# vovw/algonauts-2025

Hardware: AMD Instinct MI355X
Metric: TRs/sec trimodal encode to 1000 parcels (higher is better)
Workload: dtype bf16; 1 GPU; trimodal encode, precomputed bf16 feats, per GPU B=64 sequences (4 subjects x R=16) x T=1024, L*D=4096 per modality, hidden 3072, 8 layers, V=1000 parcels, n_output_timesteps=1024; forward only; global_batch=64, seq_len=1024, parallelism=dp1

## Files before the change

### algonauts-2025_amd/csrc/attention.hip

```cpp
#include "attn_common.h"
#include "attn_acc_regs.h"
#include "host_plan.h"

namespace {

template <int DH>
struct AttnCfg {
  static constexpr int NSUB = DH <= 64 ? 4 : (DH <= 128 ? 2 : 1);
  static constexpr int KS = DH / 32;
  static constexpr int DT = DH / 16;
  static constexpr int ROWB = DH * 2;
  static constexpr int KV = 32 * NSUB;
  static constexpr int TILE_BYTES = KV * ROWB;
  static constexpr int CHUNKS = DH / 8;
  static constexpr int WAVES = 8;
  static constexpr int PIECES = KV * CHUNKS / 64;
  static constexpr int PPW = (PIECES + WAVES - 1) / WAVES;
  static constexpr int SWZ_MASK = (CHUNKS % 16 == 0) ? 15 : 7;
  static constexpr int NBUF = DH >= 192 ? 3 : 2;
  static constexpr int SMEM = NBUF * 2 * TILE_BYTES;
  static_assert(DH % 64 == 0, "dim_head must be a multiple of 64");
};

template <int DH>
// ... 117 lines not shown
#pragma unroll
        for (int j = 0; j < 8; ++j) sv[u][j] = -INFINITY;
        continue;
      }
      f32x4_t s0 = {0.f, 0.f, 0.f, 0.f}, s1 = {0.f, 0.f, 0.f, 0.f};
#pragma unroll
      for (int ks = 0; ks < C::KS; ++ks) {
        const int off = k_rd[ks % KRD] + (ks / KRD) * SEG * 16 + u * 32 * C::ROWB;
        const bf16x8_t ka = *(const bf16x8_t*)(kt + off);
        const bf16x8_t kb2 = *(const bf16x8_t*)(kt + off + 16 * C::ROWB);
        s0 = __builtin_amdgcn_mfma_f32_16x16x32_bf16(ka, qf[ks], s0, 0, 0, 0);
        s1 = __builtin_amdgcn_mfma_f32_16x16x32_bf16(kb2, qf[ks], s1, 0, 0, 0);
      }
      const int key_base = sub_key0 + 4 * fq;
      if (RELKEY) {
        const float* qrow_e = a.qe + ((int64_t)b * T + qrow) * a.ld_qe + h * a.qe_stride_h + a.rel_left;
#pragma unroll
        for (int r = 0; r < 4; ++r) {
          int d0 = key_base + r - qrow, d1 = key_base + 16 + r - qrow;
          d0 = d0 < -a.rel_left ? -a.rel_left : (d0 > a.rel_right ? a.rel_right : d0);
          d1 = d1 < -a.rel_left ? -a.rel_left : (d1 > a.rel_right ? a.rel_right : d1);
          s0[r] += qrow_e[d0];
          s1[r] += qrow_e[d1];
        }
      }
      const bool edge = sub_key0 + 32 > T || (CAUSAL && sub_key0 + 31 > q0);
      if (edge) {
#pragma unroll
        for (int r = 0; r < 4; ++r) {
          sv[u][r] = (key_base + r < lim) ? s0[r] : -INFINITY;
          sv[u][4 + r] = (key_base + 16 + r < lim) ? s1[r] : -INFINITY;
        }
      } else {
#pragma unroll
        for (int r = 0; r < 4; ++r) { sv[u][r] = s0[r]; sv[u][4 + r] = s1[r]; }
      }
      pmax = fmaxf(pmax, fmaxf(sv[u][0], sv[u][4]));
#pragma unroll
      for (int r = 1; r < 4; ++r) pmax = max3f(pmax, sv[u][r], sv[u][4 + r]);
    }
    pmax = fmaxf(pmax, __shfl_xor(pmax, 16, 64));
    pmax = fmaxf(pmax, __shfl_xor(pmax, 32, 64));
    pmax *= scale_log2e;
    if (!__all(pmax - m_run <= 8.0f)) {
      const float m_new = fmaxf(m_run, pmax);
      const float alpha = __builtin_amdgcn_exp2f(m_run - m_new);
      m_run = m_new;
      l_run *= alpha;
      if (LSUM_MFMA) {
#pragma unroll
        for (int r = 0; r < 4; ++r) lacc[r] *= alpha;
      }
#pragma unroll
      for (int dt = 0; dt < C::DT; ++dt)
#pragma unroll
        for (int r = 0; r < 4; ++r) o[dt][r] *= alpha;
    }
    bf16x8_t pf[C::NSUB];
    float psum = 0.f;
#pragma unroll
    for (int u = 0; u < C::NSUB; ++u)
#pragma unroll
      for (int j = 0; j < 8; ++j) {
        const float p = __builtin_amdgcn_exp2f(fmaf(sv[u][j], scale_log2e, -m_run));
        if (!LSUM_MFMA) psum += p;
        pf[u][j] = (short)f32_to_bf16(p);
      }
    l_run += psum;

#pragma unroll
    for (int u = 0; u < C::NSUB; ++u) {
      const int sub_key0 = t * C::KV + u * 32;
      if (sub_key0 >= T || (CAUSAL && sub_key0 > q0 + 15)) continue;
      if (LSUM_MFMA) lacc = __builtin_amdgcn_mfma_f32_16x16x32_bf16(ones, pf[u], lacc, 0, 0, 0);
#pragma unroll
      for (int dt = 0; dt < C::DT; ++dt) {
        const int off = v_rd[dt % VRD] + (dt / VRD) * SEG * 16 + u * 32 * C::ROWB;
        const s16x4_t lo = __builtin_amdgcn_ds_read_tr16_b64_v4i16((__attribute__((address_space(3))) s16x4_t*)(vt + off));
        const s16x4_t hi =
            __builtin_amdgcn_ds_read_tr16_b64_v4i16((__attribute__((address_space(3))) s16x4_t*)(vt + off + 16 * C::ROWB));
        bf16x8_t vf;
#pragma unroll
        for (int e = 0; e < 4; ++e) { vf[e] = lo[e]; vf[4 + e] = hi[e]; }
        o[dt] = __builtin_amdgcn_mfma_f32_16x16x32_bf16(vf, pf[u], o[dt], 0, 0, 0);
      }
    }
    }
    if (C::NBUF == 3) {
      asm volatile("s_waitcnt lgkmcnt(0)" ::: "memory");
      if (t + 2 < ntiles) { stage((t + 2) % C::NBUF, (t + 2) * C::KV); wait_keep_one_tile(); }
      else { asm volatile("s_waitcnt vmcnt(0)" ::: "memory"); }
      __builtin_amdgcn_s_barrier();
    } else {
      asm volatile("s_waitcnt vmcnt(0)" ::: "memory");
      __syncthreads();
    }
  }

  float l_tot;
  if (LSUM_MFMA) {
    l_tot = lacc[0];
  } else {
    l_tot = l_run + __shfl_xor(l_run, 16, 64);
    l_tot += __shfl_xor(l_tot, 32, 64);
  }
  const float inv = 1.0f / l_tot;
  const int q = q0 + l15;
  if (q < T) {
    unsigned short* orow = a.out + ((int64_t)b * T + q) * a.ld_out + (int64_t)h * DH + 4 * fq;
#pragma unroll
    for (int dt = 0; dt < C::DT; ++dt) {
      u16x4_t pk;
#pragma unroll
      for (int e = 0; e < 4; ++e) pk[e] = f32_to_bf16(o[dt][e] * inv);
      *(u16x4_t*)(orow + 16 * dt) = pk;
    }
  }
}


struct WideCfg {
  static constexpr int DH = 384, KS = 24, DT = 12, ROWB = 768, KV = 32, CHUNKS = 48;
  static constexpr int TILE_BYTES = KV * ROWB;
  static constexpr int WAVES = 4, PPW = 6;
  static constexpr int K_SLOTS = 2, V_SLOTS = 4;
  static constexpr int V_BASE = K_SLOTS * TILE_BYTES;
  static constexpr int SMEM = (K_SLOTS + V_SLOTS) * TILE_BYTES;
  static constexpr int DEPTH = 6;
};

__device__ __forceinline__ int swz_wide(int chunk, int row) {
  return (chunk & ~15) | ((chunk ^ (((row & 3) << 2) | ((row >> 2) & 3))) & 15);
}


__device__ __forceinline__ void mfma_s_first(f32x16_t& acc, const bf16x8_t& a, const bf16x8_t& b) {
  asm volatile("v_mfma_f32_32x32x16_bf16 %0, %1, %2, 0" : "=&v"(acc) : "v"(a), "v"(b));
}
__device__ __forceinline__ void mfma_s(f32x16_t& acc, const bf16x8_t& a, const bf16x8_t& b) {
  asm volatile("v_mfma_f32_32x32x16_bf16 %0, %1, %2, %0" : "+v"(acc) : "v"(a), "v"(b));
}


__global__ __launch_bounds__(256, 1) void attn_fwd_wide384_kernel(const AttnArgs a) {
  using C = WideCfg;
  extern __shared__ __attribute__((aligned(16))) char smem[];
  const int tid = threadIdx.x, lane = tid & 63;
  const int wave = __builtin_amdgcn_readfirstlane(tid >> 6);
  const int r31 = lane & 31, h = lane >> 5;

  const int T = a.T;
  const float scale_log2e = a.scale_log2e;
  const int xcd = blockIdx.x & 7, slot = blockIdx.x >> 3;
  const int qb = slot % a.qblocks;
  const int pair = (slot / a.qblocks) * 8 + xcd;
  if (pair >= a.n_bh) return;
  const int hd = pair % a.heads_q;
  const int b = pair / a.heads_q;
  const int hk = hd / a.group;
  const int64_t ld = a.ld_kv;
  const unsigned short* qbase = a.q + (int64_t)b * T * a.ld_q + (int64_t)hd * C::DH;
  const unsigned short* kbase = a.k + (int64_t)b * T * ld + (int64_t)hk * C::DH;
  const unsigned short* vbase = a.v + (int64_t)b * T * ld + (int64_t)hk * C::DH;

  const int q0 = qb * 128 + wave * 32;
  const int qrow = (q0 + r31 < T) ? q0 + r31 : T - 1;
  bf16x8_t qf[C::KS];
#pragma unroll
  for (int ks = 0; ks < C::KS; ++ks) qf[ks] = *(const bf16x8_t*)(qbase + (int64_t)qrow * a.ld_q + ks * 16 + h * 8);
  if (a.q_cos) {
    const int half = a.q_rot_dim >> 1;
    const float* cr = a.q_cos + (int64_t)qrow * half;
    const float* sr = a.q_sin + (int64_t)qrow * half;
#pragma unroll
    for (int ks = 0; ks < C::KS; ++ks) {
      const int d0 = ks * 16 + h * 8;
      if (d0 < a.q_rot_dim) {
        const float4 c4 = *(const float4*)(cr + (d0 >> 1)), s4 = *(const float4*)(sr + (d0 >> 1));
        const float cs[4] = {c4.x, c4.y, c4.z, c4.w}, sn[4] = {s4.x, s4.y, s4.z, s4.w};
#pragma unroll
        for (int pp = 0; pp < 4; ++pp) {
          const float qa = bf16_to_f32((unsigned short)qf[ks][2 * pp]), qb = bf16_to_f32((unsigned short)qf[ks][2 * pp + 1]);
          qf[ks][2 * pp] = (short)f32_to_bf16(qa * cs[pp] - qb * sn[pp]);
          qf[ks][2 * pp + 1] = (short)f32_to_bf16(qb * cs[pp] + qa * sn[pp]);
        }
      }
    }
  }

  int st_row[C::PPW], st_src[C::PPW], st_off[C::PPW];
#pragma unroll
  for (int i = 0; i < C::PPW; ++i) {
    const int p = (wave + C::WAVES * i) * 64 + lane;
    st_row[i] = p / C::CHUNKS;
    st_src[i] = swz_wide(p % C::CHUNKS, st_row[i]) * 8;
    st_off[i] = st_row[i] * (int)ld + st_src[i];
  }
  const unsigned lds0_u = __builtin_amdgcn_readfirstlane(lds_addr(smem));
  auto stage_piece = [&](int which, int slot, int key0, int i) {
    const char* sbase = (const char*)((which ? vbase : kbase) + (int64_t)key0 * ld);
    const int piece = wave + C::WAVES * i;
    unsigned voff = (unsigned)st_off[i] * 2u;
    if (key0 + C::KV > T) {
      const int row = (key0 + st_row[i] < T) ? st_row[i] : T - 1 - key0;
      voff = (unsigned)(row * (int)ld + st_src[i]) * 2u;
    }
    const unsigned dst = lds0_u + (which ? C::V_BASE : 0) + slot * C::TILE_BYTES + piece * 1024;
    asm volatile("s_mov_b32 m0, %0\n\ts_nop 0\n\tglobal_load_lds_dwordx4 %1, %2" : : "s"(dst), "v"(voff), "s"(sbase) : "memory");
  };
  auto stage = [&](int which, int slot, int key0) {
#pragma unroll
    for (int i = 0; i < C::PPW; ++i) stage_piece(which, slot, key0, i);
  };

  int kb_off[8];
#pragma unroll
  for (int i = 0; i < 8; ++i) kb_off[i] = r31 * C::ROWB + swz_wide(2 * i + h, r31) * 16;
  const int tq = (lane & 15) >> 2, tp = lane & 3, g1 = (lane >> 4) & 1;
  int vb_off[4][2];
#pragma unroll
  for (int i = 0; i < 4; ++i)
#pragma unroll
    for (int lh = 0; lh < 2; ++lh) {
      const int row = 4 * h + tq + 8 * lh;
      vb_off[i][lh] = C::V_BASE + row * C::ROWB + swz_wide(4 * i + 2 * g1 + (tp >> 1), row) * 16 + (tp & 1) * 8;
    }
  auto ld_k = [&](const int (&ka)[8], int ks) -> bf16x8_t {
    return *(const bf16x8_t*)(smem + ka[ks & 7] + (ks >> 3) * 256);
  };
  auto ld_v = [&](const int (&va)[4][2], int i) -> bf16x8_t {
    const int s = i / C::DT, dt = i % C::DT;
    const int imm = (dt >> 2) * 256 + s * 16 * C::ROWB;
    const s16x4_t lo = __builtin_amdgcn_ds_read_tr16_b64_v4i16((__attribute__((address_space(3))) s16x4_t*)(smem + va[dt & 3][0] + imm));
    const s16x4_t hi = __builtin_amdgcn_ds_read_tr16_b64_v4i16((__attribute__((address_space(3))) s16x4_t*)(smem + va[dt & 3][1] + imm));
    bf16x8_t vf;
#pragma unroll
    for (int e = 0; e < 4; ++e) { vf[e] = lo[e]; vf[4 + e] = hi[e]; }
    return vf;
  };

  static_for<0, C::DT>([&](auto dt) { AccTile<decltype(dt)::value>::zero(); });
  float m_run = -INFINITY, l_run = 0.f;

  const int ntiles = (T + C::KV - 1) / C::KV;
  stage(0, 0, 0); stage(1, 0, 0);
  if (ntiles > 1) { stage(0, 1, C::KV); stage(1, 1, C::KV); asm volatile("s_waitcnt vmcnt(12)" ::: "memory"); }
  else { asm volatile("s_waitcnt vmcnt(0)" ::: "memory"); }
  __builtin_amdgcn_s_barrier();

  bf16x8_t kf[C::KS], vf[2 * C::DT];
  int ka[8], va[4][2];
#pragma unroll
  for (int i = 0; i < 8; ++i) ka[i] = kb_off[i];
#pragma unroll
  for (int i = 0; i < 4; ++i) { va[i][0] = vb_off[i][0]; va[i][1] = vb_off[i][1]; }
#pragma unroll
  for (int d = 0; d < C::DEPTH; ++d) kf[d] = ld_k(ka, d);

#ifdef TRIBE_ATTN_STAMPS
  unsigned long long ts0 = 0, ts1 = 0, ts2 = 0, ts3 = 0, ts4 = 0, ts5 = 0;
  unsigned long long stamp_acc[5] = {0, 0, 0, 0, 0};
#endif
  int vcur = 0;
  for (int t = 0; t < ntiles; ++t) {
    ATTN_STAMP(ts0);
    const bool more = t + 2 < ntiles;
    const int vnext2 = (vcur + 2) & 3;

    f32x16_t s;
#pragma unroll
    for (int ks = 0; ks < C::KS; ++ks) {
      if (ks + C::DEPTH < C::KS) kf[ks + C::DEPTH] = ld_k(ka, ks + C::DEPTH);
      else vf[ks + C::DEPTH - C::KS] = ld_v(va, ks + C::DEPTH - C::KS);
      if (ks % 4 == 1) { if (more) stage_piece(1, vnext2, (t + 2) * C::KV, ks / 4); }
      __builtin_amdgcn_sched_barrier(0);
      if (ks == 0) mfma_s_first(s, kf[ks], qf[ks]);
      else mfma_s(s, kf[ks], qf[ks]);
      __builtin_amdgcn_sched_barrier(0);
    }
    asm volatile("s_nop 11" : "+v"(s));
    ATTN_STAMP(ts1);

    if ((t + 1) * C::KV > T) {
#pragma unroll
      for (int r = 0; r < 16; ++r)
        if (t * C::KV + (r & 3) + 8 * (r >> 2) + 4 * h >= T) s[r] = -INFINITY;
    }
    float pmax = max3f(s[0], s[1], s[2]);
#pragma unroll
    for (int r = 3; r < 15; r += 2) pmax = max3f(pmax, s[r], s[r + 1]);
    pmax = fmaxf(pmax, s[15]);
    pmax = pair_max(pmax) * scale_log2e;
    if (!__all(pmax - m_run <= 8.0f)) {
      const float m_new = fmaxf(m_run, pmax);
      const float alpha = __builtin_amdgcn_exp2f(m_run - m_new);
      m_run = m_new;
      l_run *= alpha;
      if (t > 0) {
        asm volatile("s_nop 15\n\ts_nop 7" ::: "memory");
        static_for<0, C::DT>([&](auto dt) { AccTile<decltype(dt)::value>::scale(alpha); });
        asm volatile("s_nop 7" ::: "memory");
      }
    }
    bf16x8_t pf[2];
    float psum = 0.f;
#pragma unroll
    for (int r = 0; r < 16; ++r) {
      const float p = __builtin_amdgcn_exp2f(fmaf(s[r], scale_log2e, -m_run));
      psum += p;
      pf[r >> 3][r & 7] = (short)f32_to_bf16(p);
    }
    l_run += psum;

    ATTN_STAMP(ts2);
    if (more) asm volatile("s_waitcnt vmcnt(6)" ::: "memory");
    else asm volatile("s_waitcnt vmcnt(0)" ::: "memory");
    ATTN_STAMP(ts3);
    __builtin_amdgcn_s_barrier();
    ATTN_STAMP(ts4);
    const int kslot = t & 1;
    const int kstep = kslot ? -C::TILE_BYTES : C::TILE_BYTES;
#pragma unroll
    for (int i = 0; i < 8; ++i) asm volatile("v_add_u32 %0, %1, %0" : "+v"(ka[i]) : "s"(kstep));
    asm volatile("s_nop 1" : "+v"(pf[0]), "+v"(pf[1]));

    static_for<0, 2 * C::DT>([&](auto ic) {
      constexpr int i = decltype(ic)::value;
      if constexpr (i + C::DEPTH < 2 * C::DT) vf[i + C::DEPTH] = ld_v(va, i + C::DEPTH);
      else kf[i + C::DEPTH - 2 * C::DT] = ld_k(ka, i + C::DEPTH - 2 * C::DT);
      if constexpr (i % 4 == 1) { if (more) stage_piece(0, kslot, (t + 2) * C::KV, i / 4); }
      __builtin_amdgcn_sched_barrier(0);
      AccTile<i % C::DT>::mfma(vf[i], pf[i / C::DT]);
      __builtin_amdgcn_sched_barrier(0);
    });
    const int vstep = (vcur == 3) ? -3 * C::TILE_BYTES : C::TILE_BYTES;
#pragma unroll
    for (int i = 0; i < 4; ++i) {
      asm volatile("v_add_u32 %0, %1, %0" : "+v"(va[i][0]) : "s"(vstep));
      asm volatile("v_add_u32 %0, %1, %0" : "+v"(va[i][1]) : "s"(vstep));
    }
    vcur = (vcur + 1) & 3;
    ATTN_STAMP(ts5);
    ATTN_STAMP_ADD(0, ts0, ts1); ATTN_STAMP_ADD(1, ts1, ts2); ATTN_STAMP_ADD(2, ts2, ts3); ATTN_STAMP_ADD(3, ts3, ts4); ATTN_STAMP_ADD(4, ts4, ts5);
  }
#ifdef TRIBE_ATTN_STAMPS
  if (a.qe != nullptr && lane == 0) {
    unsigned long long* dbg = (unsigned long long*)a.qe + ((size_t)blockIdx.x * 4 + wave) * 8;
    for (int i = 0; i < 5; ++i) dbg[i] = stamp_acc[i];
    dbg[5] = (unsigned long long)ntiles;
  }
#endif

  asm volatile("s_nop 15\n\ts_nop 7" ::: "memory");
  const float l_tot = pair_sum(l_run);
  const float inv = 1.0f / l_tot;
  const int q = q0 + r31;
  if (a.lse != nullptr && h == 0 && q < T) a.lse[((int64_t)b * a.heads_q + hd) * T + q] = m_run + __builtin_amdgcn_logf(l_tot);
  unsigned short* orow = a.out + ((int64_t)b * T + (q < T ? q : T - 1)) * a.ld_out + (int64_t)hd * C::DH + 4 * h;
  static_for<0, C::DT>([&](auto dtc) {
    constexpr int dt = decltype(dtc)::value;
    float ov[16];
    AccTile<dt>::read(ov);
    if (q < T) {
#pragma unroll
      for (int g = 0; g < 4; ++g) {
        u16x4_t pk;
#pragma unroll
        for (int e = 0; e < 4; ++e) pk[e] = f32_to_bf16(ov[4 * g + e] * inv);
        *(u16x4_t*)(orow + 32 * dt + 8 * g) = pk;
      }
    }
  });
}

struct KSplitCfg {
  static constexpr int DH = 384, ROWB = 768, KV = 32, CHUNKS = 48;
  static constexpr int KS = 12, NT = 6, Q_AGPR = 8;
  static constexpr int TILE_BYTES = KV * ROWB;
  static constexpr int WAVES = 8, PPW = 6;
  static constexpr int SLOTS = 5;
  static constexpr int X_BASE = SLOTS * TILE_BYTES;
  static constexpr int SMEM = X_BASE + WAVES * 4096;
  static constexpr int DEPTH = 4;
};

__global__ __launch_bounds__(512, 2) void attn_fwd_ksplit384_kernel(const AttnArgs a) {
  using C = KSplitCfg;
  extern __shared__ __attribute__((aligned(16))) char smem[];
  const int tid = threadIdx.x, lane = tid & 63;
  const int wave = __builtin_amdgcn_readfirstlane(tid >> 6);
  const int qj = wave & 3, c = wave >> 2;
  const int r31 = lane & 31, h = lane >> 5;

  const int T = a.T;
  const float scale_log2e = a.scale_log2e;
  const int xcd = blockIdx.x & 7, slot = blockIdx.x >> 3;
  const int qb = slot % a.qblocks;
  const int pair = (slot / a.qblocks) * 8 + xcd;
  if (pair >= a.n_bh) return;
  const int hd = pair % a.heads_q;
  const int b = pair / a.heads_q;
  const int hk = hd / a.group;
  const int64_t ld = a.ld_kv;
  const unsigned short* qbase = a.q + (int64_t)b * T * a.ld_q + (int64_t)hd * C::DH;
  const unsigned short* kbase = a.k + (int64_t)b * T * ld + (int64_t)hk * C::DH;
  const unsigned short* vbase = a.v + (int64_t)b * T * ld + (int64_t)hk * C::DH;

  const int q0 = qb * 128 + qj * 32;
  const int qrow = (q0 + r31 < T) ? q0 + r31 : T - 1;
  bf16x8_t qv[C::KS - C::Q_AGPR];
  static_for<0, C::KS>([&](auto kc) {
    constexpr int k = decltype(kc)::value;
    const int ksg = 8 * (k >> 2) + 4 * c + (k & 3);
    const bf16x8_t qfrag = *(const bf16x8_t*)(qbase + (int64_t)qrow * a.ld_q + ksg * 16 + h * 8);
    if constexpr (k < C::Q_AGPR) QFrag<k>::set(qfrag);
    else qv[k - C::Q_AGPR] = qfrag;
  });
  static_for<0, C::NT>([&](auto n) { AccTile<decltype(n)::value>::zero(); });
  asm volatile("s_nop 7" ::: "memory");

  int st_off[C::PPW];
#pragma unroll
  for (int i = 0; i < C::PPW; ++i) {
    const int p = (qj + 4 * i) * 64 + lane;
    st_off[i] = (p / C::CHUNKS) * (int)ld + swz_wide(p % C::CHUNKS, p / C::CHUNKS) * 8;
  }
  const unsigned short* my_base = c ? vbase : kbase;
  auto stage_piece = [&](int slot_i, int key0, int i) {
    const unsigned short* src = my_base + (int64_t)key0 * ld;
    const int piece = qj + 4 * i;
    int off = st_off[i];
    if (key0 + C::KV > T) {
      const int p = piece * 64 + lane;
      const int row0 = p / C::CHUNKS;
      const int row = (key0 + row0 < T) ? row0 : T - 1 - key0;
      off = row * (int)ld + swz_wide(p % C::CHUNKS, row0) * 8;
    }
    glds16(src + off, lds_addr(smem) + slot_i * C::TILE_BYTES + piece * 1024);
  };

  int ka[4];
#pragma unroll
  for (int i = 0; i < 4; ++i) ka[i] = r31 * C::ROWB + swz_wide(8 * c + 2 * i + h, r31) * 16;
  const int tq = (lane & 15) >> 2, tp = lane & 3, g1 = (lane >> 4) & 1;
  int va[2][2];
#pragma unroll
  for (int e = 0; e < 2; ++e)
#pragma unroll
    for (int lh = 0; lh < 2; ++lh) {
      const int row = 4 * h + tq + 8 * lh;
      va[e][lh] = C::TILE_BYTES + row * C::ROWB + swz_wide(4 * (2 * c + e) + 2 * g1 + (tp >> 1), row) * 16 + (tp & 1) * 8;
    }
  auto ld_k = [&](int k) -> bf16x8_t { return *(const bf16x8_t*)(smem + ka[k & 3] + (k >> 2) * 256); };
  auto ld_v = [&](int i) -> bf16x8_t {
    const int sk = i / C::NT, n = i % C::NT;
    const int imm = (n >> 1) * 256 + sk * 16 * C::ROWB;
    const s16x4_t lo = __builtin_amdgcn_ds_read_tr16_b64_v4i16((__attribute__((address_space(3))) s16x4_t*)(smem + va[n & 1][0] + imm));
    const s16x4_t hi = __builtin_amdgcn_ds_read_tr16_b64_v4i16((__attribute__((address_space(3))) s16x4_t*)(smem + va[n & 1][1] + imm));
    bf16x8_t vf;
#pragma unroll
    for (int e = 0; e < 4; ++e) { vf[e] = lo[e]; vf[4 + e] = hi[e]; }
    return vf;
  };
  const int x_mine = C::X_BASE + wave * 4096 + lane * 16, x_peer = C::X_BASE + (wave ^ 4) * 4096 + lane * 16;

  float m_run = -INFINITY, l_run = 0.f;
  const int ntiles = (T + C::KV - 1) / C::KV;
  auto stage_half = [&](int hh) {
    if ((hh & 1) != c) return;
#pragma unroll
    for (int i = 0; i < C::PPW; ++i) stage_piece(hh % C::SLOTS, (hh >> 1) * C::KV, i);
  };
  const int nhalf = 2 * ntiles;
  for (int hh = 0; hh < C::SLOTS && hh < nhalf; ++hh) stage_half(hh);
  if (c == 0) {
    if (ntiles >= 3) asm volatile("s_waitcnt vmcnt(12)" ::: "memory");
    else if (ntiles == 2) asm volatile("s_waitcnt vmcnt(6)" ::: "memory");
    else asm volatile("s_waitcnt vmcnt(0)" ::: "memory");
  }
  __builtin_amdgcn_s_barrier();

  bf16x8_t kf[C::KS], vf[2 * C::NT];
#pragma unroll
  for (int d = 0; d < C::DEPTH; ++d) kf[d] = ld_k(d);

  int kslot = 0, vslot = 1;
  for (int t = 0; t < ntiles; ++t) {
    f32x16_t s;
    static_for<0, C::KS>([&](auto kc) {
      constexpr int k = decltype(kc)::value;
#ifndef TRIBE_ATTN_DMA_ONLY
      if constexpr (k + C::DEPTH < C::KS) kf[k + C::DEPTH] = ld_k(k + C::DEPTH);
#endif
      if constexpr (k % 2 == 1) { if (c == 0 && t >= 1 && t + 2 < ntiles) stage_piece((2 * t + 4) % C::SLOTS, (t + 2) * C::KV, k / 2); }
      __builtin_amdgcn_sched_barrier(0);
#ifndef TRIBE_ATTN_DMA_ONLY
      if constexpr (k == 0) QFrag<k>::mfma_first(s, kf[k]);
      else if constexpr (k < C::Q_AGPR) QFrag<k>::mfma(s, kf[k]);
      else mfma_s(s, kf[k], qv[k - C::Q_AGPR]);
#else
      if constexpr (k == 0) { for (int r = 0; r < 16; ++r) s[r] = (float)r31; }
#endif
      __builtin_amdgcn_sched_barrier(0);
    });
    asm volatile("s_nop 11" : "+v"(s));
#pragma unroll
    for (int q4 = 0; q4 < 4; ++q4) *(f32x4_t*)(smem + x_mine + q4 * 1024) = f32x4_t{s[4 * q4], s[4 * q4 + 1], s[4 * q4 + 2], s[4 * q4 + 3]};
    if (c == 0 ? (t + 2 < ntiles) : (t + 1 < ntiles)) asm volatile("s_waitcnt vmcnt(6) lgkmcnt(0)" ::: "memory");
    else asm volatile("s_waitcnt vmcnt(0) lgkmcnt(0)" ::: "memory");
    __builtin_amdgcn_s_barrier();
#pragma unroll
    for (int d = 0; d < C::DEPTH; ++d) vf[d] = ld_v(d);
#pragma unroll
    for (int q4 = 0; q4 < 4; ++q4) {
      const f32x4_t o4 = *(const f32x4_t*)(smem + x_peer + q4 * 1024);
#pragma unroll
      for (int e = 0; e < 4; ++e) s[4 * q4 + e] += o4[e];
    }

    if ((t + 1) * C::KV > T) {
#pragma unroll
      for (int r = 0; r < 16; ++r)
        if (t * C::KV + (r & 3) + 8 * (r >> 2) + 4 * h >= T) s[r] = -INFINITY;
    }
    float pmax = max3f(s[0], s[1], s[2]);
#pragma unroll
    for (int r = 3; r < 15; r += 2) pmax = max3f(pmax, s[r], s[r + 1]);
    pmax = fmaxf(pmax, s[15]);
    pmax = pair_max(pmax) * scale_log2e;
    if (!__all(pmax - m_run <= 8.0f)) {
      const float m_new = fmaxf(m_run, pmax);
      const float alpha = __builtin_amdgcn_exp2f(m_run - m_new);
      m_run = m_new;
      l_run *= alpha;
      if (t > 0) {
        asm volatile("s_nop 15\n\ts_nop 7" ::: "memory");
        static_for<0, C::NT>([&](auto n) { AccTile<decltype(n)::value>::scale(alpha); });
        asm volatile("s_nop 7" ::: "memory");
      }
    }
    bf16x8_t pf[2];
    float psum = 0.f;
#pragma unroll
    for (int r = 0; r < 16; ++r) {
      const float p = __builtin_amdgcn_exp2f(fmaf(s[r], scale_log2e, -m_run));
      psum += p;
      pf[r >> 3][r & 7] = (short)f32_to_bf16(p);
    }
    l_run += psum;

    const int knext = kslot + 2 >= C::SLOTS ? kslot + 2 - C::SLOTS : kslot + 2;
    const int kstep = (knext - kslot) * C::TILE_BYTES;
#pragma unroll
    for (int i = 0; i < 4; ++i) asm volatile("v_add_u32 %0, %1, %0" : "+v"(ka[i]) : "s"(kstep));
    asm volatile("s_nop 1" : "+v"(pf[0]), "+v"(pf[1]));

    static_for<0, 2 * C::NT>([&](auto ic) {
      constexpr int i = decltype(ic)::value;
#ifndef TRIBE_ATTN_DMA_ONLY
      if constexpr (i + C::DEPTH < 2 * C::NT) vf[i + C::DEPTH] = ld_v(i + C::DEPTH);
      else kf[i + C::DEPTH - 2 * C::NT] = ld_k(i + C::DEPTH - 2 * C::NT);
#endif
      if constexpr (i % 2 == 1) { if (c == 1 && t + 2 < ntiles) stage_piece(kslot, (t + 2) * C::KV, i / 2); }
      __builtin_amdgcn_sched_barrier(0);
#ifndef TRIBE_ATTN_DMA_ONLY
      AccTile<i % C::NT>::mfma(vf[i], pf[i / C::NT]);
#endif
      __builtin_amdgcn_sched_barrier(0);
    });
    const int vnext = vslot + 2 >= C::SLOTS ? vslot + 2 - C::SLOTS : vslot + 2;
    const int vstep = (vnext - vslot) * C::TILE_BYTES;
#pragma unroll
    for (int e = 0; e < 2; ++e) {
      asm volatile("v_add_u32 %0, %1, %0" : "+v"(va[e][0]) : "s"(vstep));
      asm volatile("v_add_u32 %0, %1, %0" : "+v"(va[e][1]) : "s"(vstep));
    }
    kslot = knext;
    vslot = vnext;
    __builtin_amdgcn_s_barrier();
  }

  asm volatile("s_nop 15\n\ts_nop 7" ::: "memory");
  const float inv = 1.0f / pair_sum(l_run);
  const int q = q0 + r31;
  unsigned short* orow = a.out + ((int64_t)b * T + (q < T ? q : T - 1)) * a.ld_out + (int64_t)hd * C::DH + 4 * h + 64 * c;
  static_for<0, C::NT>([&](auto nc) {
    constexpr int n = decltype(nc)::value;
    float ov[16];
    AccTile<n>::read(ov);
    if (q < T) {
#pragma unroll
      for (int g = 0; g < 4; ++g) {
        u16x4_t pk;
#pragma unroll
        for (int e = 0; e < 4; ++e) pk[e] = f32_to_bf16(ov[4 * g + e] * inv);
        *(u16x4_t*)(orow + 128 * (n >> 1) + 32 * (n & 1) + 8 * g) = pk;
      }
    }
  });
}

int launch_attn_ksplit384(const AttnArgs& a, int64_t B, hipStream_t s) {
  using C = KSplitCfg;
  static bool attr_done = false;
  if (!attr_done) {
    (void)hipFuncSetAttribute((const void*)attn_fwd_ksplit384_kernel, hipFuncAttributeMaxDynamicSharedMemorySize, C::SMEM);
    attr_done = true;
  }
  const int64_t nblocks = (B * a.heads_q + 7) / 8 * 8 * a.qblocks;
  if (nblocks >= (1ll << 31)) { tribe_set_error("tribe_attention_fwd: grid too large"); return -1; }
  if ((int64_t)a.T * a.ld_kv >= (1ll << 31)) { tribe_set_error("tribe_attention_fwd: sequence too long for 32-bit offsets"); return -1; }
  hipLaunchKernelGGL(attn_fwd_ksplit384_kernel, dim3((unsigned)nblocks), dim3(512), C::SMEM, s, a);
  TRIBE_LAUNCH_CHECK();
  return 0;
}

int launch_attn_wide384(const AttnArgs& a, int64_t B, hipStream_t s) {
  using C = WideCfg;
  static bool attr_done = false;
  if (!attr_done) {
    (void)hipFuncSetAttribute((const void*)attn_fwd_wide384_kernel, hipFuncAttributeMaxDynamicSharedMemorySize, C::SMEM);
    attr_done = true;
  }
  const int64_t nblocks = (B * a.heads_q + 7) / 8 * 8 * a.qblocks;
  if (nblocks >= (1ll << 31)) { tribe_set_error("tribe_attention_fwd: grid too large"); return -1; }
  if ((int64_t)a.T * a.ld_kv >= (1ll << 31)) { tribe_set_error("tribe_attention_fwd: sequence too long for 32-bit offsets"); return -1; }
  hipLaunchKernelGGL(attn_fwd_wide384_kernel, dim3((unsigned)nblocks), dim3(256), C::SMEM, s, a);
  TRIBE_LAUNCH_CHECK();
  return 0;
}

template <int DH, int CAUSAL, int RELKEY>
int launch_attn(const AttnArgs& a, int64_t B, hipStream_t s) {
  using C = AttnCfg<DH>;
  static bool attr_done = false;
  if (!attr_done) {
    (void)hipFuncSetAttribute((const void*)attn_fwd_kernel<DH, CAUSAL, RELKEY>, hipFuncAttributeMaxDynamicSharedMemorySize, C::SMEM);
    attr_done = true;
  }
  const int64_t nblocks = (B * a.heads_q + 7) / 8 * 8 * a.qblocks;
  if (nblocks >= (1ll << 31)) { tribe_set_error("tribe_attention_fwd: grid too large"); return -1; }
  if ((int64_t)a.T * a.ld_kv >= (1ll << 31)) { tribe_set_error("tribe_attention_fwd: sequence too long for 32-bit offsets"); return -1; }
  hipLaunchKernelGGL((attn_fwd_kernel<DH, CAUSAL, RELKEY>), dim3((unsigned)nblocks), dim3(512), C::SMEM, s, a);
  TRIBE_LAUNCH_CHECK();
  return 0;
}

}
int tribe_internal_attn_d64_launch(const void* args, int64_t B, int relkey, int variant, hipStream_t s);
namespace {

int g_attn_d64_variant = 0;
int g_attn_wide384 = 1;

template <int DH>
int launch_attn_dh(const AttnArgs& a, int64_t B, int causal, hipStream_t s) {
  if (DH == 384 && !causal && g_attn_wide384 == 1) return launch_attn_wide384(a, B, s);
  if (DH == 384 && !causal && g_attn_wide384 == 2) return launch_attn_ksplit384(a, B, s);
  return causal ? launch_attn<DH, 1, 0>(a, B, s) : launch_attn<DH, 0, 0>(a, B, s);
}

}

void tribe_internal_attention_set_wide384(int on) { g_attn_wide384 = on; }
void tribe_internal_attention_set_d64_variant(int v) { g_attn_d64_variant = v; }

int tribe_internal_attention_fused_supported(int dim_head) {
  return dim_head == 64 || dim_head == 128 || dim_head == 192 || dim_head == 384;
}

static int attention_dispatch_impl(const tribe_attention_desc* d, const float* q_cos, const float* q_sin, int q_rot_dim, void* stream);
static int attention_dispatch(const tribe_attention_desc* d, const float* q_cos, const float* q_sin, int q_rot_dim, void* stream) {
  const double flops = d ? 4.0 * (double)d->T * (double)d->dim_head * (double)d->T * (double)d->heads_q * (double)d->B * (d->causal ? 0.5 : 1.0) : 0.0;
  const int slot = tribe_internal_prof_before(TRIBE_ROLE_ATTENTION, flops, (hipStream_t)stream);
  const int rc = attention_dispatch_impl(d, q_cos, q_sin, q_rot_dim, stream);
  tribe_internal_prof_after(slot, (hipStream_t)stream);
  return rc;
}
static int attention_dispatch_impl(const tribe_attention_desc* d, const float* q_cos, const float* q_sin, int q_rot_dim, void* stream) {
  TRIBE_REQUIRE(d && d->q && d->k && d->v && d->out, "tribe_attention_fwd_ex: null pointer");
  TRIBE_REQUIRE(d->B > 0 && d->T > 0 && d->heads_q > 0 && d->heads_kv > 0 && d->heads_q % d->heads_kv == 0,
                "tribe_attention_fwd_ex: bad shape (B=%lld T=%lld heads %d/%d)", (long long)d->B, (long long)d->T, d->heads_q, d->heads_kv);
  TRIBE_REQUIRE(tribe_internal_attention_fused_supported(d->dim_head), "tribe_attention_fwd_ex: dim_head=%d not in {64,128,192,384}",
                d->dim_head);
  TRIBE_REQUIRE(d->ld_k == d->ld_v, "tribe_attention_fwd_ex: k and v must share their row stride");
  TRIBE_REQUIRE(d->ld_q % 8 == 0 && d->ld_k % 8 == 0 && d->ld_out % 4 == 0 && ((uintptr_t)d->q % 16) == 0 && ((uintptr_t)d->k % 16) == 0 &&
                    ((uintptr_t)d->v % 16) == 0 && ((uintptr_t)d->out % 8) == 0,
                "tribe_attention_fwd_ex: operands must be 16-byte aligned with row strides that are multiples of 8");
  AttnArgs a;
  a.q = d->q; a.k = d->k; a.v = d->v; a.out = d->out;
  a.ld_q = d->ld_q; a.ld_kv = d->ld_k; a.ld_out = d->ld_out;
  a.T = (int)d->T; a.heads_q = d->heads_q; a.group = d->heads_q / d->heads_kv;
  a.scale_log2e = d->scale * 1.4426950408889634f;
  a.qblocks = (int)((d->T + 127) / 128);
  a.n_bh = (int)(d->B * d->heads_q);
  a.qe = d->rel_qe; a.ld_qe = d->ld_rel_qe; a.qe_stride_h = d->rel_stride_h; a.rel_left = d->rel_left; a.rel_right = d->rel_right;
  a.q_cos = q_cos; a.q_sin = q_sin; a.q_rot_dim = q_rot_dim;
  a.lse = d->lse;
  TRIBE_REQUIRE(!d->lse || (tribe_attention_lse_supported(d->dim_head, d->causal) && !d->rel_qe),
                "tribe_attention_fwd_ex: the log-sum-exp output exists for dim_head 384, bidirectional, default mode only");
  hipStream_t s = (hipStream_t)stream;
#ifdef TRIBE_ATTN_STAMPS
  if (d->rel_qe && d->dim_head == 384) return launch_attn_dh<384>(a, d->B, d->causal, s);
  if (d->rel_qe && d->dim_head == 64 && d->rel_left < 0) return tribe_internal_attn_d64_launch(&a, d->B, 0, g_attn_d64_variant, s);
#endif
  if (d->rel_qe) {
    TRIBE_REQUIRE(d->dim_head == 64 && !d->causal, "tribe_attention_fwd_ex: the relative_key bias is built for dim_head 64, non-causal");
    TRIBE_REQUIRE(d->rel_left >= 0 && d->rel_right >= 0 && d->rel_stride_h >= d->rel_left + d->rel_right + 1 &&
                      d->ld_rel_qe >= (int64_t)d->heads_q * d->rel_stride_h,
                  "tribe_attention_fwd_ex: bad relative_key table geometry");
    return g_attn_wide384 ? tribe_internal_attn_d64_launch(&a, d->B, 1, g_attn_d64_variant, s) : launch_attn<64, 0, 1>(a, d->B, s);
  }
  switch (d->dim_head) {
    case 64: return (!d->causal && g_attn_wide384) ? tribe_internal_attn_d64_launch(&a, d->B, 0, g_attn_d64_variant, s) : launch_attn_dh<64>(a, d->B, d->causal, s);
    case 128: return launch_attn_dh<128>(a, d->B, d->causal, s);
    case 192: return launch_attn_dh<192>(a, d->B, d->causal, s);
    default: return launch_attn_dh<384>(a, d->B, d->causal, s);
  }
}

extern "C" int tribe_attention_fwd_ex(const tribe_attention_desc* d, void* stream) { return attention_dispatch(d, nullptr, nullptr, 0, stream); }

extern "C" int tribe_attention_lse_supported(int32_t dim_head, int32_t causal) { return dim_head == 384 && !causal && g_attn_wide384 == 1; }

int tribe_internal_attention_rotates_q(int dim_head) { return dim_head == 384 && g_attn_wide384 == 1; }

static tribe_attention_desc fused_desc(const uint16_t* qkv, int64_t B, int64_t T, int heads, int dim_head, float scale, uint16_t* out) {
  const int64_t inner = (int64_t)heads * dim_head;
  tribe_attention_desc d = attn_zero();
  d.q = qkv; d.k = qkv + inner; d.v = qkv + 2 * inner;
  d.ld_q = d.ld_k = d.ld_v = 3 * inner;
  d.out = out; d.ld_out = inner;
  d.B = B; d.T = T; d.heads_q = heads; d.heads_kv = heads; d.dim_head = dim_head; d.scale = scale;
  return d;
}

int tribe_internal_attention_fused_qrot(const uint16_t* qkv, int64_t B, int64_t T, int heads, int dim_head, float scale, uint16_t* out,
                                        const float* cos_tab, const float* sin_tab, int rot_dim, hipStream_t s) {
  TRIBE_REQUIRE(tribe_internal_attention_rotates_q(dim_head) && cos_tab && sin_tab && rot_dim > 0 && rot_dim % 16 == 0 && rot_dim <= dim_head,
                "tribe_internal_attention_fused_qrot: unsupported configuration");
  const tribe_attention_desc d = fused_desc(qkv, B, T, heads, dim_head, scale, out);
  return attention_dispatch(&d, cos_tab, sin_tab, rot_dim, (void*)s);
}

int tribe_internal_attention_fused(const uint16_t* qkv, int64_t B, int64_t T, int heads, int dim_head, float scale, uint16_t* out,
                                   hipStream_t s) {
  const tribe_attention_desc d = fused_desc(qkv, B, T, heads, dim_head, scale, out);
  return attention_dispatch(&d, nullptr, nullptr, 0, (void*)s);
}

extern "C" int tribe_debug_attention_qrot(const uint16_t* qkv, int64_t B, int64_t T, int32_t heads, int32_t dim_head, float scale,
                                          uint16_t* out, const float* cos_tab, const float* sin_tab, int32_t rot_dim, void* stream) {
  TRIBE_REQUIRE(qkv && out && B > 0 && T > 0 && heads > 0, "tribe_debug_attention_qrot: null pointer or bad shape");
  return tribe_internal_attention_fused_qrot(qkv, B, T, heads, dim_head, scale, out, cos_tab, sin_tab, rot_dim, (hipStream_t)stream);
}
```

### algonauts-2025_amd/csrc/attn_common.h

```cpp
#pragma once
#include "gemm_common.h"
#include <utility>

namespace {

typedef __attribute__((ext_vector_type(4))) short s16x4_t;

__device__ __forceinline__ float max3f(float a, float b, float c) {
  float d;
  asm("v_max3_f32 %0, %1, %2, %3" : "=v"(d) : "v"(a), "v"(b), "v"(c));
  return d;
}

__device__ __forceinline__ void glds16(const void* gsrc, unsigned lds_dst) {
  unsigned keep;
  asm volatile("s_mov_b32 %0, m0\n\ts_mov_b32 m0, %2\n\ts_nop 0\n\tglobal_load_lds_dwordx4 %1, off\n\ts_mov_b32 m0, %0"
               : "=&s"(keep) : "v"(gsrc), "s"(lds_dst) : "memory");
}
__device__ __forceinline__ unsigned lds_addr(const void* p) { return (unsigned)(uintptr_t)(lptr_t)p; }

struct AttnArgs {
  const unsigned short* q; const unsigned short* k; const unsigned short* v;
  unsigned short* out;
  int64_t ld_q, ld_kv, ld_out;
  int T, heads_q, group;
  float scale_log2e;
  int qblocks;
  int n_bh;
  const float* qe; int64_t ld_qe; int qe_stride_h; int rel_left, rel_right;
  const float* q_cos; const float* q_sin; int q_rot_dim;
  float* lse;
};

template <int I, int N, class F>
__device__ __forceinline__ void static_for(F&& f) {
  if constexpr (I < N) {
    f(std::integral_constant<int, I>{});
    static_for<I + 1, N>(f);
  }
}

__device__ __forceinline__ void pair_split(float x, float& lo, float& hi) {
  lo = x;
  hi = x;
  asm volatile("s_nop 1\n\tv_permlane32_swap_b32 %0, %1" : "+v"(lo), "+v"(hi));
}
__device__ __forceinline__ float pair_max(float x) {
  float lo, hi;
  pair_split(x, lo, hi);
  return fmaxf(lo, hi);
}
__device__ __forceinline__ float pair_sum(float x) {
  float lo, hi;
  pair_split(x, lo, hi);
  return lo + hi;
}

}

#ifdef TRIBE_ATTN_STAMPS
#define ATTN_STAMP(var)                                                                   \
  do {                                                                                    \
    __builtin_amdgcn_sched_barrier(0);                                                    \
    asm volatile("s_memtime %0\n\ts_waitcnt lgkmcnt(0)" : "=s"(var)::"memory");           \
    __builtin_amdgcn_sched_barrier(0);                                                    \
  } while (0)
#define ATTN_STAMP_ADD(i, a, b) stamp_acc[i] += (b) - (a)
#else
#define ATTN_STAMP(var) do {} while (0)
#define ATTN_STAMP_ADD(i, a, b) do {} while (0)
#endif
```

Measured before the change: 638,800 TRs/s.

## Chain multiple query blocks per attention workgroup and widen output stores

```diff
diff --git a/algonauts-2025_amd/csrc/attention.hip b/algonauts-2025_amd/csrc/attention.hip
--- a/algonauts-2025_amd/csrc/attention.hip
+++ b/algonauts-2025_amd/csrc/attention.hip
@@ -293,9 +293,10 @@
   const int T = a.T;
   const float scale_log2e = a.scale_log2e;
   const int xcd = blockIdx.x & 7, slot = blockIdx.x >> 3;
-  const int qb = slot % a.qblocks;
-  const int pair = (slot / a.qblocks) * 8 + xcd;
+  const int qb0 = (slot % a.qgroups) * a.qchain;
+  const int pair = (slot / a.qgroups) * 8 + xcd;
   if (pair >= a.n_bh) return;
+  const int nblk = (a.qblocks - qb0 < a.qchain) ? a.qblocks - qb0 : a.qchain;
   const int hd = pair % a.heads_q;
   const int b = pair / a.heads_q;
   const int hk = hd / a.group;
@@ -303,31 +304,43 @@
   const unsigned short* qbase = a.q + (int64_t)b * T * a.ld_q + (int64_t)hd * C::DH;
   const unsigned short* kbase = a.k + (int64_t)b * T * ld + (int64_t)hk * C::DH;
   const unsigned short* vbase = a.v + (int64_t)b * T * ld + (int64_t)hk * C::DH;
-
-  const int q0 = qb * 128 + wave * 32;
-  const int qrow = (q0 + r31 < T) ? q0 + r31 : T - 1;
+#ifdef TRIBE_ATTN_STAMPS
+  unsigned long long te0 = 0, te1 = 0, te2 = 0, te3 = 0, te4 = 0, te5 = 0, te6 = 0;
+  unsigned long long edge_acc[6] = {0, 0, 0, 0, 0, 0};
+  ATTN_STAMP(te0);
+#endif
+
+  auto opaque_lane = [](int x) { asm volatile("" : "+v"(x)); return x; };
+  auto query_row = [&](int qb) { const int q = qb * 128 + wave * 32 + opaque_lane(r31); return q < T ? q : T - 1; };
   bf16x8_t qf[C::KS];
-#pragma unroll
-  for (int ks = 0; ks < C::KS; ++ks) qf[ks] = *(const bf16x8_t*)(qbase + (int64_t)qrow * a.ld_q + ks * 16 + h * 8);
-  if (a.q_cos) {
+  auto load_q = [&](int qb) {
+    const unsigned short* qr = qbase + (int64_t)query_row(qb) * a.ld_q + opaque_lane(h) * 8;
+#pragma unroll
+    for (int ks = 0; ks < C::KS; ++ks) qf[ks] = *(const bf16x8_t*)(qr + ks * 16);
+  };
+  auto rotate_q = [&](int qb) {
+    if (!a.q_cos) return;
+    const int qrow = query_row(qb);
     const int half = a.q_rot_dim >> 1;
     const float* cr = a.q_cos + (int64_t)qrow * half;
     const float* sr = a.q_sin + (int64_t)qrow * half;
+    const int h8 = opaque_lane(h) * 8;
 #pragma unroll
     for (int ks = 0; ks < C::KS; ++ks) {
-      const int d0 = ks * 16 + h * 8;
+      const int d0 = ks * 16 + h8;
       if (d0 < a.q_rot_dim) {
         const float4 c4 = *(const float4*)(cr + (d0 >> 1)), s4 = *(const float4*)(sr + (d0 >> 1));
         const float cs[4] = {c4.x, c4.y, c4.z, c4.w}, sn[4] = {s4.x, s4.y, s4.z, s4.w};
 #pragma unroll
         for (int pp = 0; pp < 4; ++pp) {
-          const float qa = bf16_to_f32((unsigned short)qf[ks][2 * pp]), qb = bf16_to_f32((unsigned short)qf[ks][2 * pp + 1]);
-          qf[ks][2 * pp] = (short)f32_to_bf16(qa * cs[pp] - qb * sn[pp]);
-          qf[ks][2 * pp + 1] = (short)f32_to_bf16(qb * cs[pp] + qa * sn[pp]);
+          const float qa = bf16_to_f32((unsigned short)qf[ks][2 * pp]), qb_ = bf16_to_f32((unsigned short)qf[ks][2 * pp + 1]);
+          qf[ks][2 * pp] = (short)f32_to_bf16(qa * cs[pp] - qb_ * sn[pp]);
+          qf[ks][2 * pp + 1] = (short)f32_to_bf16(qb_ * cs[pp] + qa * sn[pp]);
         }
       }
     }
-  }
+  };
+  load_q(qb0);
 
   int st_row[C::PPW], st_src[C::PPW], st_off[C::PPW];
 #pragma unroll
@@ -380,14 +393,26 @@
     return vf;
   };
 
-  static_for<0, C::DT>([&](auto dt) { AccTile<decltype(dt)::value>::zero(); });
-  float m_run = -INFINITY, l_run = 0.f;
-
   const int ntiles = (T + C::KV - 1) / C::KV;
   stage(0, 0, 0); stage(1, 0, 0);
+#ifdef TRIBE_ATTN_STAMPS
+  if (ntiles > 1) {
+    stage(0, 1, C::KV); stage(1, 1, C::KV);
+    ATTN_STAMP(te5);
+    asm volatile("s_waitcnt vmcnt(24)" ::: "memory");
+    ATTN_STAMP(te6);
+    edge_acc[4] += te5 - te0;
+    edge_acc[5] += te6 - te5;
+    asm volatile("s_waitcnt vmcnt(12)" ::: "memory");
+  } else { asm volatile("s_waitcnt vmcnt(0)" ::: "memory"); }
+  __builtin_amdgcn_s_barrier();
+  ATTN_STAMP(te1);
+  edge_acc[0] += te1 - te0;
+#else
   if (ntiles > 1) { stage(0, 1, C::KV); stage(1, 1, C::KV); asm volatile("s_waitcnt vmcnt(12)" ::: "memory"); }
   else { asm volatile("s_waitcnt vmcnt(0)" ::: "memory"); }
   __builtin_amdgcn_s_barrier();
+#endif
 
   bf16x8_t kf[C::KS], vf[2 * C::DT];
   int ka[8], va[4][2];
@@ -403,9 +428,26 @@
   unsigned long long stamp_acc[5] = {0, 0, 0, 0, 0};
 #endif
   int vcur = 0;
+  int kslot = 0;
+  int tiles_left = nblk * ntiles;
+  for (int blk = 0; blk < nblk; ++blk) {
+#ifdef TRIBE_ATTN_STAMPS
+  if (blk > 0) ATTN_STAMP(te1);
+  asm volatile("s_waitcnt vmcnt(0)" ::: "memory");
+#endif
+  rotate_q(qb0 + blk);
+  static_for<0, C::DT>([&](auto dt) { AccTile<decltype(dt)::value>::zero(); });
+  asm volatile("s_nop 7" ::: "memory");
+  float m_run = -INFINITY, l_run = 0.f;
+  int qwarm = 0;
+#ifdef TRIBE_ATTN_STAMPS
+  ATTN_STAMP(te2);
+  edge_acc[1] += te2 - te1;
+#endif
   for (int t = 0; t < ntiles; ++t) {
     ATTN_STAMP(ts0);
-    const bool more = t + 2 < ntiles;
+    const bool more = tiles_left > 2;
+    const int key2 = ((t + 2 < ntiles) ? t + 2 : t + 2 - ntiles) * C::KV;
     const int vnext2 = (vcur + 2) & 3;
 
     f32x16_t s;
@@ -413,7 +455,7 @@
     for (int ks = 0; ks < C::KS; ++ks) {
       if (ks + C::DEPTH < C::KS) kf[ks + C::DEPTH] = ld_k(ka, ks + C::DEPTH);
       else vf[ks + C::DEPTH - C::KS] = ld_v(va, ks + C::DEPTH - C::KS);
-      if (ks % 4 == 1) { if (more) stage_piece(1, vnext2, (t + 2) * C::KV, ks / 4); }
+      if (ks % 4 == 1) { if (more) stage_piece(1, vnext2, key2, ks / 4); }
       __builtin_amdgcn_sched_barrier(0);
       if (ks == 0) mfma_s_first(s, kf[ks], qf[ks]);
       else mfma_s(s, kf[ks], qf[ks]);
@@ -459,17 +501,21 @@
     ATTN_STAMP(ts3);
     __builtin_amdgcn_s_barrier();
     ATTN_STAMP(ts4);
-    const int kslot = t & 1;
     const int kstep = kslot ? -C::TILE_BYTES : C::TILE_BYTES;
 #pragma unroll
     for (int i = 0; i < 8; ++i) asm volatile("v_add_u32 %0, %1, %0" : "+v"(ka[i]) : "s"(kstep));
     asm volatile("s_nop 1" : "+v"(pf[0]), "+v"(pf[1]));
+    if (t == ntiles - 1 && tiles_left > 1) {
+      const unsigned short* qr = qbase + (int64_t)query_row(qb0 + blk + 1) * a.ld_q + opaque_lane(h) * 192;
+      qwarm = *(const int*)qr | *(const int*)(qr + 64) | *(const int*)(qr + 128);
+    }
+    __builtin_amdgcn_sched_barrier(0);
 
     static_for<0, 2 * C::DT>([&](auto ic) {
       constexpr int i = decltype(ic)::value;
       if constexpr (i + C::DEPTH < 2 * C::DT) vf[i + C::DEPTH] = ld_v(va, i + C::DEPTH);
       else kf[i + C::DEPTH - 2 * C::DT] = ld_k(ka, i + C::DEPTH - 2 * C::DT);
-      if constexpr (i % 4 == 1) { if (more) stage_piece(0, kslot, (t + 2) * C::KV, i / 4); }
+      if constexpr (i % 4 == 1) { if (more) stage_piece(0, kslot, key2, i / 4); }
       __builtin_amdgcn_sched_barrier(0);
       AccTile<i % C::DT>::mfma(vf[i], pf[i / C::DT]);
       __builtin_amdgcn_sched_barrier(0);
@@ -481,37 +527,75 @@
       asm volatile("v_add_u32 %0, %1, %0" : "+v"(va[i][1]) : "s"(vstep));
     }
     vcur = (vcur + 1) & 3;
+    kslot ^= 1;
+    --tiles_left;
     ATTN_STAMP(ts5);
     ATTN_STAMP_ADD(0, ts0, ts1); ATTN_STAMP_ADD(1, ts1, ts2); ATTN_STAMP_ADD(2, ts2, ts3); ATTN_STAMP_ADD(3, ts3, ts4); ATTN_STAMP_ADD(4, ts4, ts5);
   }
 #ifdef TRIBE_ATTN_STAMPS
-  if (a.qe != nullptr && lane == 0) {
-    unsigned long long* dbg = (unsigned long long*)a.qe + ((size_t)blockIdx.x * 4 + wave) * 8;
-    for (int i = 0; i < 5; ++i) dbg[i] = stamp_acc[i];
-    dbg[5] = (unsigned long long)ntiles;
-  }
-#endif
+  ATTN_STAMP(te3);
+  edge_acc[2] += te3 - te2;
+#endif
+
+  asm volatile("" : : "v"(qwarm));
+  if (tiles_left > 0) load_q(qb0 + blk + 1);
 
   asm volatile("s_nop 15\n\ts_nop 7" ::: "memory");
   const float l_tot = pair_sum(l_run);
   const float inv = 1.0f / l_tot;
-  const int q = q0 + r31;
-  if (a.lse != nullptr && h == 0 && q < T) a.lse[((int64_t)b * a.heads_q + hd) * T + q] = m_run + __builtin_amdgcn_logf(l_tot);
-  unsigned short* orow = a.out + ((int64_t)b * T + (q < T ? q : T - 1)) * a.ld_out + (int64_t)hd * C::DH + 4 * h;
-  static_for<0, C::DT>([&](auto dtc) {
-    constexpr int dt = decltype(dtc)::value;
-    float ov[16];
-    AccTile<dt>::read(ov);
-    if (q < T) {
-#pragma unroll
-      for (int g = 0; g < 4; ++g) {
-        u16x4_t pk;
-#pragma unroll
-        for (int e = 0; e < 4; ++e) pk[e] = f32_to_bf16(ov[4 * g + e] * inv);
-        *(u16x4_t*)(orow + 32 * dt + 8 * g) = pk;
-      }
-    }
-  });
+  const int q = (qb0 + blk) * 128 + wave * 32 + opaque_lane(r31);
+  const int ho = opaque_lane(h);
+  if (a.lse != nullptr && ho == 0 && q < T) a.lse[((int64_t)b * a.heads_q + hd) * T + q] = m_run + __builtin_amdgcn_logf(l_tot);
+  unsigned short* orow = a.out + ((int64_t)b * T + (q < T ? q : T - 1)) * a.ld_out + (int64_t)hd * C::DH;
+  if (a.st16) {
+    static_for<0, C::DT>([&](auto dtc) {
+      constexpr int dt = decltype(dtc)::value;
+      float ov[16];
+      AccTile<dt>::read(ov);
+#pragma unroll
+      for (int j = 0; j < 2; ++j) {
+        unsigned x[2], y[2];
+#pragma unroll
+        for (int w = 0; w < 2; ++w) {
+          x[w] = (unsigned)f32_to_bf16(ov[8 * j + 2 * w] * inv) | ((unsigned)f32_to_bf16(ov[8 * j + 2 * w + 1] * inv) << 16);
+          y[w] = (unsigned)f32_to_bf16(ov[8 * j + 4 + 2 * w] * inv) | ((unsigned)f32_to_bf16(ov[8 * j + 4 + 2 * w + 1] * inv) << 16);
+          asm volatile("s_nop 1\n\tv_permlane32_swap_b32 %0, %1" : "+v"(x[w]), "+v"(y[w]));
+        }
+        if (q < T) *(u32x4_t*)(orow + 32 * dt + 16 * j + 8 * ho) = u32x4_t{x[0], x[1], y[0], y[1]};
+      }
+    });
+  } else {
+    static_for<0, C::DT>([&](auto dtc) {
+      constexpr int dt = decltype(dtc)::value;
+      float ov[16];
+      AccTile<dt>::read(ov);
+      if (q < T) {
+#pragma unroll
+        for (int g = 0; g < 4; ++g) {
+          u16x4_t pk;
+#pragma unroll
+          for (int e = 0; e < 4; ++e) pk[e] = f32_to_bf16(ov[4 * g + e] * inv);
+          *(u16x4_t*)(orow + 4 * ho + 32 * dt + 8 * g) = pk;
+        }
+      }
+    });
+  }
+#ifdef TRIBE_ATTN_STAMPS
+  ATTN_STAMP(te4);
+  edge_acc[3] += te4 - te3;
+#endif
+  }
+#ifdef TRIBE_ATTN_STAMPS
+  if (a.qe != nullptr && lane == 0) {
+    unsigned long long* dbg = (unsigned long long*)a.qe + ((size_t)blockIdx.x * 4 + wave) * 16;
+    for (int i = 0; i < 5; ++i) dbg[i] = stamp_acc[i];
+    dbg[5] = (unsigned long long)ntiles * nblk;
+    for (int i = 0; i < 4; ++i) dbg[6 + i] = edge_acc[i];
+    dbg[10] = (unsigned long long)nblk;
+    dbg[11] = edge_acc[4];
+    dbg[12] = edge_acc[5];
+  }
+#endif
 }
 
 struct KSplitCfg {
@@ -756,14 +840,53 @@
   return 0;
 }
 
-int launch_attn_wide384(const AttnArgs& a, int64_t B, hipStream_t s) {
+#ifndef TRIBE_ATTN_QCHAIN_MAX
+#define TRIBE_ATTN_QCHAIN_MAX 2
+#endif
+#ifndef TRIBE_ATTN_CHAIN_DEFAULT
+#define TRIBE_ATTN_CHAIN_DEFAULT 0
+#endif
+#ifndef TRIBE_ATTN_STORE16
+#define TRIBE_ATTN_STORE16 1
+#endif
+int attn_qchain_policy(int64_t n_bh, int qblocks, int cus) {
+  if (n_bh <= 0 || qblocks <= 0 || cus <= 0) return 1;
+  for (int c = TRIBE_ATTN_QCHAIN_MAX; c > 1; c >>= 1) {
+    if (c > qblocks) continue;
+    const int64_t groups = (qblocks + c - 1) / c;
+    if (n_bh * groups >= 2 * (int64_t)cus) return c;
+  }
+  return 1;
+}
+
+int g_attn_qchain = TRIBE_ATTN_CHAIN_DEFAULT ? 0 : 1;
+
+int device_cus() {
+  static int cus[64] = {};
+  int dev = 0;
+  (void)hipGetDevice(&dev);
+  if (dev < 0 || dev >= 64) dev = 0;
+  if (!cus[dev]) {
+    int n = 0;
+    if (hipDeviceGetAttribute(&n, hipDeviceAttributeMultiprocessorCount, dev) != hipSuccess || n <= 0) n = 256;
+    cus[dev] = n;
+  }
+  return cus[dev];
+}
+
+int launch_attn_wide384(const AttnArgs& a_in, int64_t B, hipStream_t s) {
   using C = WideCfg;
   static bool attr_done = false;
   if (!attr_done) {
     (void)hipFuncSetAttribute((const void*)attn_fwd_wide384_kernel, hipFuncAttributeMaxDynamicSharedMemorySize, C::SMEM);
     attr_done = true;
   }
-  const int64_t nblocks = (B * a.heads_q + 7) / 8 * 8 * a.qblocks;
+  AttnArgs a = a_in;
+  a.qchain = g_attn_qchain ? g_attn_qchain : attn_qchain_policy(B * a.heads_q, a.qblocks, device_cus());
+  if (a.qchain > a.qblocks) a.qchain = a.qblocks;
+  a.qgroups = (a.qblocks + a.qchain - 1) / a.qchain;
+  a.st16 = TRIBE_ATTN_STORE16 && ((uintptr_t)a.out % 16) == 0 && a.ld_out % 8 == 0;
+  const int64_t nblocks = (B * a.heads_q + 7) / 8 * 8 * a.qgroups;
   if (nblocks >= (1ll << 31)) { tribe_set_error("tribe_attention_fwd: grid too large"); return -1; }
   if ((int64_t)a.T * a.ld_kv >= (1ll << 31)) { tribe_set_error("tribe_attention_fwd: sequence too long for 32-bit offsets"); return -1; }
   hipLaunchKernelGGL(attn_fwd_wide384_kernel, dim3((unsigned)nblocks), dim3(256), C::SMEM, s, a);
@@ -838,6 +961,7 @@
   a.qe = d->rel_qe; a.ld_qe = d->ld_rel_qe; a.qe_stride_h = d->rel_stride_h; a.rel_left = d->rel_left; a.rel_right = d->rel_right;
   a.q_cos = q_cos; a.q_sin = q_sin; a.q_rot_dim = q_rot_dim;
   a.lse = d->lse;
+  a.qchain = 1; a.qgroups = a.qblocks; a.st16 = 0;
   TRIBE_REQUIRE(!d->lse || (tribe_attention_lse_supported(d->dim_head, d->causal) && !d->rel_qe),
                 "tribe_attention_fwd_ex: the log-sum-exp output exists for dim_head 384, bidirectional, default mode only");
   hipStream_t s = (hipStream_t)stream;
@@ -895,3 +1019,10 @@
   TRIBE_REQUIRE(qkv && out && B > 0 && T > 0 && heads > 0, "tribe_debug_attention_qrot: null pointer or bad shape");
   return tribe_internal_attention_fused_qrot(qkv, B, T, heads, dim_head, scale, out, cos_tab, sin_tab, rot_dim, (hipStream_t)stream);
 }
+
+extern "C" int tribe_debug_attention_set_qchain(int32_t qchain) {
+  TRIBE_REQUIRE(qchain == 0 || qchain == 1 || qchain == 2 || qchain == 4, "tribe_debug_attention_set_qchain: %d not in {0, 1, 2, 4}", qchain);
+  g_attn_qchain = qchain ? qchain : (TRIBE_ATTN_CHAIN_DEFAULT ? 0 : 1);
+  return 0;
+}
+extern "C" int tribe_debug_attention_qchain_for(int64_t n_bh, int32_t qblocks, int32_t cus) { return attn_qchain_policy(n_bh, qblocks, cus); }
diff --git a/algonauts-2025_amd/csrc/attn_common.h b/algonauts-2025_amd/csrc/attn_common.h
--- a/algonauts-2025_amd/csrc/attn_common.h
+++ b/algonauts-2025_amd/csrc/attn_common.h
@@ -5,6 +5,7 @@
 namespace {
 
 typedef __attribute__((ext_vector_type(4))) short s16x4_t;
+typedef __attribute__((ext_vector_type(4))) unsigned u32x4_t;
 
 __device__ __forceinline__ float max3f(float a, float b, float c) {
   float d;
@@ -30,6 +31,7 @@
   const float* qe; int64_t ld_qe; int qe_stride_h; int rel_left, rel_right;
   const float* q_cos; const float* q_sin; int q_rot_dim;
   float* lse;
+  int qchain, qgroups, st16;
 };
 
 template <int I, int N, class F>
```

Result: no change. 640,800 TRs/s, median of 6 (+0.3%).
